# dmMaze/comic-text-detector

Hardware: AMD Instinct MI355X
Metric: pages/sec at 1024x1024 bs=32 (end-to-end detector, device-resident pages) (higher is better)
Workload: dtype f16

## Files before the change

comic-text-detector_amd/csrc/kernels.h:

```cpp
#pragma once
#include <vector>

#include "ctd_common.h"

void launch_conv_direct(const ConvArgs& a, bool f16, hipStream_t st);
void launch_convt_direct(const ConvArgs& a, bool f16, hipStream_t st);
void launch_input_nchw(const float* in, void* dst, int pitch, int B, int H, int W, bool f16, hipStream_t st);
void launch_input_u8(const uint8_t* in, void* dst, int pitch, int B, int H, int W, bool f16, hipStream_t st);
void launch_maxpool(const void* src, int pitchS, void* dst, int pitchD, int C, int B, int H, int W, int k,
                    bool f16, hipStream_t st);
bool sppf_pool3_supported(int pitch, int slot, int C, int H, int W, int k, const void* cat, int esize = 2);
void launch_sppf_pool3(void* cat, int pitch, int slot, int C, int B, int H, int W, int k, hipStream_t st, int esize = 2);
void launch_avgpool2(const void* src, int pitchS, void* dst, int pitchD, int C, int B, int Ho, int Wo,
                     bool f16, hipStream_t st);
void launch_detect_decode(const void* raw, int pitch, bool raw_f16, float* blks, int rows_total, int row_off,
                          int B, int ny, int nx, int na, int no, float stride, const float* anchors_px,
                          hipStream_t st);
void launch_export_plane(const void* src, int pitch, bool f16, float* out, int nplanes, int plane, uint8_t* u8,
                         int u8_mode, float thresh, int B, int H, int W, hipStream_t st);

void launch_db_step(const float* lines, float k, float* out, uint8_t* bitmap, float thresh, int B, int H, int W,
                    hipStream_t st);

extern int g_tail_max_blocks;
extern int g_igemm_force_bk;
int igemm_pick_bk(int c0, int c1, int K, int N, int log2_down);
void igemm_pack_weights(const float* logical, int nphase, int N, int K, int bn, int bk, bool tiled,
                        std::vector<half_t>& out);
bool igemm_supported(const ConvArgs& a);
int igemm_ntile(int N);
const char* launch_conv_igemm(const ConvArgs& a, bool dst_f32, hipStream_t st);

int f32_mfma_ntile(int N);
bool conv_f32_mfma_supported(const ConvArgs& a);
void launch_conv_f32_mfma(const ConvArgs& a, hipStream_t st);

bool conv_split_supported(const ConvArgs& a);
const char* launch_conv_split(const ConvArgs& a, hipStream_t st);
bool stem_split_supported(const ConvArgs& a);
void launch_stem_split(const ConvArgs& a, const void* input, int in_fmt, hipStream_t st);
extern int g_split_halo;
extern long long g_split_halo_min_patches;
bool conv_split_halo_supported(const ConvArgs& a);
void launch_conv_split_halo(const ConvArgs& a, hipStream_t st);
void split_pack_weights(const float* logical, int nphase, int N, int K, int npad, std::vector<half_t>& out,
                        std::vector<float>& oscale);

extern int g_conv_halo;
bool conv_halo_supported(const ConvArgs& a, bool dst_f32);
int conv_tuning_set(const char* key, long long value);
void launch_conv_halo(const ConvArgs& a, hipStream_t st);

extern long long g_halo3;
extern long long g_halo3_min_blocks;
bool conv_halo3_supported(const ConvArgs& a, bool dst_f32);
bool conv_halo3_post_supported(const ConvArgs& a);
bool conv_halo3_segp_supported(const ConvArgs& a);
void launch_conv_halo3(const ConvArgs& a, hipStream_t st);
int halo3_tuning_set(const char* key, long long value);

struct C3Args {
  SrcView s0, s1;
  int B, H, W;
  const half_t *w12, *wm1, *wm2, *wc3;
  const float *b12, *bm1, *bm2, *bc3;
  void* dst;
  int pitchD;
  int act;
  const void* zeros;
  int prio;
  half_t* dbg;
};
extern int g_fuse;
extern long long g_c3_min_patches;
bool c3_fused_supported(const C3Args& a);
void launch_c3_fused(const C3Args& a, hipStream_t st);

struct C3bArgs {
  SrcView y1;
  SrcView y2;
  int B, H, W;
  int ch;
  const half_t *wm1, *wm2, *wc3;
  const float *bm1, *bm2, *bc3;
  void* dst;
  int pitchD;
  int act;
  int add;
  int cv3;
  int tap_major;
  const void* zeros;
  int prio;
};
extern long long g_c3b_min_patches;
extern int g_c3b_max_ch;
extern int g_c3b_cfg64, g_c3b_cfg128;
bool c3b_supported(const C3bArgs& a);
const char* launch_c3b(const C3bArgs& a, hipStream_t st);

struct Stem2Args {
  const void* in; int in_fmt;
  int B, H, W;
  const half_t* wfrag; const float* bias0; int act0;
  const half_t* w1; const float* bias1; int act1;
  half_t* dst; int pitchD;
  int prio;
};
bool stem_conv2_supported(const Stem2Args& a);
void launch_stem_conv2(const Stem2Args& a, hipStream_t st);

void launch_stem(const void* in, int in_fmt, half_t* dst, int pitchD, int B, int H, int W, int N,
                 const half_t* wfrag, const float* bias, int act, hipStream_t st);
void stem_pack_weights(const float* W , std::vector<half_t>& out);
const char* launch_seg_final(const half_t* src, int pitch, int C, int B, int H, int W, const float* w, float bias,
                             float* mask, uint8_t* mask_u8, hipStream_t st);
void launch_seg_final_f32(const float* src, int pitch, int C, int B, int H, int W, const float* w, float* mask,
                          uint8_t* mask_u8, hipStream_t st);
void launch_seg_final_gather(const float* P, int B, int H, int W, float bias, float* mask, uint8_t* mask_u8, hipStream_t st);
extern int g_seg_final_mfma;
extern int g_db_up_mfma;
const char* launch_db_up(const void* src, bool f32in, int pitch, int q, int nbr, int B, int H, int W, const float* params,
                         float* lines, uint8_t* bitmap, float thresh, hipStream_t st);

size_t nms_workspace_bytes(int B, int rows);
void launch_nms(const float* blks, int B, int rows, int no, float conf, float iou, int max_det, int max_nms,
                float max_wh, float* dets, int* counts, void* ws, hipStream_t st);
size_t ccl_workspace_bytes(int B, int H, int W);
void launch_ccl(const uint8_t* img, int B, int H, int W, int thresh, int conn, int* labels, int* n_out,
                int* stats, int max_labels, void* ws, hipStream_t st, int invert = 0, int* first = nullptr, int bg_negative = 0);
void launch_ccl_dual(const uint8_t* img, int B, int H, int W, int thresh, int* labels, int* n_f, int* n_b, int* st_f,
                     int* st_b, int* first_f, int* first_b, int max_labels, void* ws, hipStream_t st);

void launch_resize_linear_u8(const uint8_t* src, int sH, int sW, int C, uint8_t* dst, int dH, int dW, int canvasH,
                             int canvasW, hipStream_t st);

void launch_region_warp(const ctd_region_job* jobs, int n, const int* tile_first, int n_tiles, uint8_t* out, hipStream_t st);
void launch_region_batches(const ctd_region_batch_job* jobs, int n, const int* tile_first, int n_tiles, const void* tables,
                           void* out, int dtype, int layout, int reverse, int pad, hipStream_t st);

void launch_mfma_probe(const half_t* a, const half_t* b, float* out, hipStream_t st);
```

comic-text-detector_amd/csrc/kernels_basic.hip:

```cpp
#include "kernels.h"

namespace {

template <typename T>
__device__ __forceinline__ const T* src_pixel(const SrcView& s, int b, int iy, int ix) {
  int sy = s.up ? (iy >> 1) : iy;
  int sx = s.up ? (ix >> 1) : ix;
  return (const T*)s.ptr + ((size_t)((size_t)b * s.H + sy) * s.W + sx) * s.pitch;
}

template <typename T, bool PRECISE>
__global__ __launch_bounds__(256) void conv_direct_kernel(ConvArgs a) {
  const long long total = (long long)a.M * a.N;
  const int Ct = a.s0.c + a.s1.c;
  const float* __restrict__ w = (const float*)a.w;
  for (long long idx = (long long)blockIdx.x * blockDim.x + threadIdx.x; idx < total;
       idx += (long long)gridDim.x * blockDim.x) {
    const int n = (int)(idx % a.N);
    const int m = (int)(idx / a.N);
    const int ox = m % a.Mw;
    const int oy = (m / a.Mw) % a.Mh;
    const int b = m / (a.Mw * a.Mh);
    float acc = 0.f;
    for (int ty = 0; ty < a.KH; ++ty) {
// ... 25 lines not shown
  const long long total = (long long)a.B * a.oH * a.oW * a.N;
  const int C = a.s0.c;
  const int k = a.KH, s = a.stride, p = a.dy0;
  const float* __restrict__ w = (const float*)a.w;
  for (long long idx = (long long)blockIdx.x * blockDim.x + threadIdx.x; idx < total;
       idx += (long long)gridDim.x * blockDim.x) {
    const int n = (int)(idx % a.N);
    const long long pix = idx / a.N;
    const int ox = (int)(pix % a.oW);
    const int oy = (int)((pix / a.oW) % a.oH);
    const int b = (int)(pix / ((long long)a.oW * a.oH));
    float acc = 0.f;
    for (int ky = 0; ky < k; ++ky) {
      const int ty = oy + p - ky;
      if (ty < 0 || (ty % s) != 0) continue;
      const int iy = ty / s;
      if (iy >= a.Hin) continue;
      for (int kx = 0; kx < k; ++kx) {
        const int tx = ox + p - kx;
        if (tx < 0 || (tx % s) != 0) continue;
        const int ix = tx / s;
        if (ix >= a.Win) continue;
        const T* p0 = src_pixel<T>(a.s0, b, iy, ix);
        const float* wp = w + (size_t)((ky * k + kx) * C) * a.N + n;
        for (int c = 0; c < C; ++c) acc = fmaf(to_f(p0[c]), wp[(size_t)c * a.N], acc);
      }
    }
    if (a.bias) acc += a.bias[n];
    acc = PRECISE ? ctd_act_precise(acc, a.act) : ctd_act(acc, a.act);
    ((T*)a.dst)[(size_t)pix * a.pitchD + n] = from_f<T>(acc);
  }
}

template <typename T>
__global__ void input_nchw_kernel(const float* __restrict__ in, T* __restrict__ dst, int pitch, int B, int H, int W) {
  const long long hw = (long long)H * W;
  const long long total = (long long)B * hw;
  for (long long i = (long long)blockIdx.x * blockDim.x + threadIdx.x; i < total;
       i += (long long)gridDim.x * blockDim.x) {
    const long long b = i / hw, p = i % hw;
    const float* src = in + b * 3 * hw + p;
    T* d = dst + i * pitch;
    d[0] = from_f<T>(src[0]);
    d[1] = from_f<T>(src[hw]);
    d[2] = from_f<T>(src[2 * hw]);
    for (int c = 3; c < pitch; ++c) d[c] = from_f<T>(0.f);
  }
}

template <typename T>
__global__ void input_u8_kernel(const uint8_t* __restrict__ in, T* __restrict__ dst, int pitch, long long total) {
  for (long long i = (long long)blockIdx.x * blockDim.x + threadIdx.x; i < total;
       i += (long long)gridDim.x * blockDim.x) {
    const uint8_t* s = in + i * 3;
    T* d = dst + i * pitch;
    d[0] = from_f<T>((float)s[0] / 255.0f);
    d[1] = from_f<T>((float)s[1] / 255.0f);
    d[2] = from_f<T>((float)s[2] / 255.0f);
    for (int c = 3; c < pitch; ++c) d[c] = from_f<T>(0.f);
  }
}

template <typename T>
__global__ void maxpool_kernel(const T* __restrict__ src, int pitchS, T* __restrict__ dst, int pitchD, int C,
                               int B, int H, int W, int k) {
  const long long total = (long long)B * H * W * C;
  const int r = k / 2;
  for (long long i = (long long)blockIdx.x * blockDim.x + threadIdx.x; i < total;
       i += (long long)gridDim.x * blockDim.x) {
    const int c = (int)(i % C);
    const long long pix = i / C;
    const int x = (int)(pix % W), y = (int)((pix / W) % H);
    const long long b = pix / ((long long)W * H);
    float m = -INFINITY;
    for (int dy = -r; dy <= r; ++dy) {
      const int yy = y + dy;
      if (yy < 0 || yy >= H) continue;
      for (int dx = -r; dx <= r; ++dx) {
        const int xx = x + dx;
        if (xx < 0 || xx >= W) continue;
        m = fmaxf(m, to_f(src[((b * H + yy) * W + xx) * pitchS + c]));
      }
    }
    dst[pix * pitchD + c] = from_f<T>(m);
  }
}

__global__ void maxpool_h8_kernel(const half_t* __restrict__ src, int pitchS, half_t* __restrict__ dst, int pitchD,
                                  int C8, int B, int H, int W, int k) {
  const long long total = (long long)B * H * W * C8;
  const int r = k / 2;
  for (long long i = (long long)blockIdx.x * blockDim.x + threadIdx.x; i < total;
       i += (long long)gridDim.x * blockDim.x) {
    const int c = (int)(i % C8) * 8;
    const long long pix = i / C8;
    const int x = (int)(pix % W), y = (int)((pix / W) % H);
    const long long b = pix / ((long long)W * H);
    half8_t m;
#pragma unroll
    for (int e = 0; e < 8; ++e) m[e] = (half_t)-65504.f;
    for (int dy = -r; dy <= r; ++dy) {
      const int yy = y + dy;
      if (yy < 0 || yy >= H) continue;
      for (int dx = -r; dx <= r; ++dx) {
        const int xx = x + dx;
        if (xx < 0 || xx >= W) continue;
        const half8_t v = *(const half8_t*)(src + ((b * H + yy) * W + xx) * pitchS + c);
#pragma unroll
        for (int e = 0; e < 8; ++e) m[e] = v[e] > m[e] ? v[e] : m[e];
      }
    }
    *(half8_t*)(dst + pix * pitchD + c) = m;
  }
}

constexpr int SPPF_LDS_BYTES = 65536;
template <typename T, typename V, int NV>
__global__ __launch_bounds__(256) void sppf_pool3_kernel(T* __restrict__ cat, int pitch, int slot, int CG, int H, int W, int r) {
  __shared__ __attribute__((aligned(16))) unsigned char sm_raw[SPPF_LDS_BYTES];
  V* A = (V*)sm_raw;
  V* Bf = A + H * W;
  const int HW = H * W;
  const int b = blockIdx.x / CG, cg = blockIdx.x - b * CG;
  T* base = cat + (size_t)b * HW * pitch + cg * NV;
  for (int p = threadIdx.x; p < HW; p += 256) A[p] = *(const V*)(base + (size_t)p * pitch);
  __syncthreads();
  auto vmax = [](V a, V b2) {
    V o;
#pragma unroll
    for (int e = 0; e < NV; ++e) o[e] = b2[e] > a[e] ? b2[e] : a[e];
    return o;
  };
  for (int lvl = 1; lvl <= 3; ++lvl) {
    for (int p = threadIdx.x; p < HW; p += 256) {
      const int y = p / W, x = p - y * W;
      V m = A[p];
      for (int dx = -r; dx <= r; ++dx)
        if (dx && (unsigned)(x + dx) < (unsigned)W) m = vmax(m, A[p + dx]);
      Bf[p] = m;
    }
    __syncthreads();
    for (int p = threadIdx.x; p < HW; p += 256) {
      const int y = p / W;
      V m = Bf[p];
      for (int dy = -r; dy <= r; ++dy)
        if (dy && (unsigned)(y + dy) < (unsigned)H) m = vmax(m, Bf[p + dy * W]);
      A[p] = m;
      *(V*)(base + (size_t)lvl * slot + (size_t)p * pitch) = m;
    }
    __syncthreads();
  }
}

template <typename T>
__global__ void avgpool2_kernel(const T* __restrict__ src, int pitchS, T* __restrict__ dst, int pitchD, int C,
                                int B, int Ho, int Wo) {
  const long long total = (long long)B * Ho * Wo * C;
  const int Wi = Wo * 2, Hi = Ho * 2;
  for (long long i = (long long)blockIdx.x * blockDim.x + threadIdx.x; i < total;
       i += (long long)gridDim.x * blockDim.x) {
    const int c = (int)(i % C);
    const long long pix = i / C;
    const int x = (int)(pix % Wo), y = (int)((pix / Wo) % Ho);
    const long long b = pix / ((long long)Wo * Ho);
    const T* p = src + ((b * Hi + 2 * y) * Wi + 2 * x) * pitchS + c;
    const float s = (to_f(p[0]) + to_f(p[pitchS])) + (to_f(p[(size_t)Wi * pitchS]) + to_f(p[(size_t)(Wi + 1) * pitchS]));
    dst[pix * pitchD + c] = from_f<T>(s * 0.25f);
  }
}

template <typename T>
__global__ void detect_decode_kernel(const T* __restrict__ raw, int pitch, float* __restrict__ blks, int rows_total,
                                     int row_off, int B, int ny, int nx, int na, int no, float stride,
                                     const float* __restrict__ anchors) {
  const long long total = (long long)B * na * ny * nx;
  for (long long i = (long long)blockIdx.x * blockDim.x + threadIdx.x; i < total;
       i += (long long)gridDim.x * blockDim.x) {
    const int x = (int)(i % nx), y = (int)((i / nx) % ny);
    const int an = (int)((i / ((long long)nx * ny)) % na);
    const long long b = i / ((long long)nx * ny * na);
    const T* p = raw + ((b * ny + y) * nx + x) * pitch + an * no;
    float* o = blks + (b * rows_total + row_off + ((long long)an * ny + y) * nx + x) * no;
    for (int j = 0; j < no; ++j) {
      const float s = 1.0f / (1.0f + expf(-to_f(p[j])));
      float v = s;
      if (j == 0) v = (s * 2.f - 0.5f + (float)x) * stride;
      else if (j == 1) v = (s * 2.f - 0.5f + (float)y) * stride;
      else if (j == 2) { const float t = s * 2.f; v = t * t * anchors[an * 2 + 0]; }
      else if (j == 3) { const float t = s * 2.f; v = t * t * anchors[an * 2 + 1]; }
      o[j] = v;
    }
  }
}

template <typename T>
__global__ void export_plane_kernel(const T* __restrict__ src, int pitch, float* __restrict__ out, int nplanes,
                                    int plane, uint8_t* __restrict__ u8, int u8_mode, float thresh, int B, int H,
                                    int W) {
  const long long hw = (long long)H * W;
  const long long total = (long long)B * hw;
  for (long long i = (long long)blockIdx.x * blockDim.x + threadIdx.x; i < total;
       i += (long long)gridDim.x * blockDim.x) {
    const long long b = i / hw, p = i % hw;
    const float v = to_f(src[i * pitch]);
    if (out) out[(b * nplanes + plane) * hw + p] = v;
    if (u8_mode == 1) u8[i] = (uint8_t)(v * 255.0f);
    else if (u8_mode == 2) u8[i] = v > thresh ? 1 : 0;
  }
}

inline int grid_for(long long total, int block = 256) {
  long long g = (total + block - 1) / block;
  if (g > 256LL * 32) g = 256LL * 32;
  if (g < 1) g = 1;
  return (int)g;
}

}

void launch_conv_direct(const ConvArgs& a, bool f16, hipStream_t st) {
  const int g = grid_for((long long)a.M * a.N);
  if (f16) hipLaunchKernelGGL((conv_direct_kernel<half_t, false>), dim3(g), dim3(256), 0, st, a);
  else hipLaunchKernelGGL((conv_direct_kernel<float, true>), dim3(g), dim3(256), 0, st, a);
}

void launch_convt_direct(const ConvArgs& a, bool f16, hipStream_t st) {
  const int g = grid_for((long long)a.B * a.oH * a.oW * a.N);
  if (f16) hipLaunchKernelGGL((convt_direct_kernel<half_t, false>), dim3(g), dim3(256), 0, st, a);
  else hipLaunchKernelGGL((convt_direct_kernel<float, true>), dim3(g), dim3(256), 0, st, a);
}

void launch_input_nchw(const float* in, void* dst, int pitch, int B, int H, int W, bool f16, hipStream_t st) {
  const int g = grid_for((long long)B * H * W);
  if (f16) hipLaunchKernelGGL((input_nchw_kernel<half_t>), dim3(g), dim3(256), 0, st, in, (half_t*)dst, pitch, B, H, W);
  else hipLaunchKernelGGL((input_nchw_kernel<float>), dim3(g), dim3(256), 0, st, in, (float*)dst, pitch, B, H, W);
}

void launch_input_u8(const uint8_t* in, void* dst, int pitch, int B, int H, int W, bool f16, hipStream_t st) {
  const long long t = (long long)B * H * W;
  const int g = grid_for(t);
  if (f16) hipLaunchKernelGGL((input_u8_kernel<half_t>), dim3(g), dim3(256), 0, st, in, (half_t*)dst, pitch, t);
  else hipLaunchKernelGGL((input_u8_kernel<float>), dim3(g), dim3(256), 0, st, in, (float*)dst, pitch, t);
}

void launch_maxpool(const void* src, int pitchS, void* dst, int pitchD, int C, int B, int H, int W, int k,
                    bool f16, hipStream_t st) {
  const int g = grid_for((long long)B * H * W * C);
  if (f16 && C % 8 == 0 && pitchS % 8 == 0 && pitchD % 8 == 0 && (((uintptr_t)src | (uintptr_t)dst) & 15) == 0)
    hipLaunchKernelGGL(maxpool_h8_kernel, dim3(grid_for((long long)B * H * W * (C / 8))), dim3(256), 0, st,
                       (const half_t*)src, pitchS, (half_t*)dst, pitchD, C / 8, B, H, W, k);
  else if (f16)
    hipLaunchKernelGGL((maxpool_kernel<half_t>), dim3(g), dim3(256), 0, st, (const half_t*)src, pitchS,
                       (half_t*)dst, pitchD, C, B, H, W, k);
  else
    hipLaunchKernelGGL((maxpool_kernel<float>), dim3(g), dim3(256), 0, st, (const float*)src, pitchS, (float*)dst,
                       pitchD, C, B, H, W, k);
}

bool sppf_pool3_supported(int pitch, int slot, int C, int H, int W, int k, const void* cat, int esize) {
  if (k != 5 && k != 3 && k != 7) return false;
  const int v = 16 / esize;
  if (C % v || pitch % v || slot % v || ((uintptr_t)cat & 15)) return false;
  return (long long)H * W * 2 * 8 <= SPPF_LDS_BYTES;
}
void launch_sppf_pool3(void* cat, int pitch, int slot, int C, int B, int H, int W, int k, hipStream_t st, int esize) {
  typedef float float2_t __attribute__((ext_vector_type(2)));
  const bool wide = (long long)H * W * 2 * 16 <= SPPF_LDS_BYTES;
  if (esize == 4) {
    if (wide)
      hipLaunchKernelGGL((sppf_pool3_kernel<float, float4_t, 4>), dim3(B * (C / 4)), dim3(256), 0, st, (float*)cat, pitch, slot, C / 4, H, W, k / 2);
    else
      hipLaunchKernelGGL((sppf_pool3_kernel<float, float2_t, 2>), dim3(B * (C / 2)), dim3(256), 0, st, (float*)cat, pitch, slot, C / 2, H, W, k / 2);
  } else if (wide) {
    hipLaunchKernelGGL((sppf_pool3_kernel<half_t, half8_t, 8>), dim3(B * (C / 8)), dim3(256), 0, st, (half_t*)cat, pitch, slot, C / 8, H, W, k / 2);
  } else {
    hipLaunchKernelGGL((sppf_pool3_kernel<half_t, half4_t, 4>), dim3(B * (C / 4)), dim3(256), 0, st, (half_t*)cat, pitch, slot, C / 4, H, W, k / 2);
  }
}

void launch_avgpool2(const void* src, int pitchS, void* dst, int pitchD, int C, int B, int Ho, int Wo, bool f16,
                     hipStream_t st) {
  const int g = grid_for((long long)B * Ho * Wo * C);
  if (f16)
    hipLaunchKernelGGL((avgpool2_kernel<half_t>), dim3(g), dim3(256), 0, st, (const half_t*)src, pitchS,
                       (half_t*)dst, pitchD, C, B, Ho, Wo);
  else
    hipLaunchKernelGGL((avgpool2_kernel<float>), dim3(g), dim3(256), 0, st, (const float*)src, pitchS, (float*)dst,
                       pitchD, C, B, Ho, Wo);
}

void launch_detect_decode(const void* raw, int pitch, bool raw_f16, float* blks, int rows_total, int row_off, int B,
                          int ny, int nx, int na, int no, float stride, const float* anchors_px, hipStream_t st) {
  const int g = grid_for((long long)B * na * ny * nx);
  if (raw_f16)
    hipLaunchKernelGGL((detect_decode_kernel<half_t>), dim3(g), dim3(256), 0, st, (const half_t*)raw, pitch, blks,
                       rows_total, row_off, B, ny, nx, na, no, stride, anchors_px);
  else
    hipLaunchKernelGGL((detect_decode_kernel<float>), dim3(g), dim3(256), 0, st, (const float*)raw, pitch, blks,
                       rows_total, row_off, B, ny, nx, na, no, stride, anchors_px);
}

__global__ void db_step_kernel(const float* __restrict__ lines, float k, float* __restrict__ out,
                               uint8_t* __restrict__ bitmap, float thresh, int B, int hw) {
  const long long total = (long long)B * hw;
  for (long long i = (long long)blockIdx.x * blockDim.x + threadIdx.x; i < total; i += (long long)gridDim.x * blockDim.x) {
    const long long b = i / hw, p = i % hw;
    const float x = lines[(b * 2) * hw + p], y = lines[(b * 2 + 1) * hw + p];
    const float v = 1.0f / (1.0f + expf(-k * (x - y)));
    out[i] = v;
    if (bitmap) bitmap[i] = v > thresh ? 1 : 0;
  }
}

void launch_db_step(const float* lines, float k, float* out, uint8_t* bitmap, float thresh, int B, int H, int W,
                    hipStream_t st) {
  hipLaunchKernelGGL(db_step_kernel, dim3(grid_for((long long)B * H * W)), dim3(256), 0, st, lines, k, out, bitmap, thresh,
                     B, H * W);
}

void launch_export_plane(const void* src, int pitch, bool f16, float* out, int nplanes, int plane, uint8_t* u8,
                         int u8_mode, float thresh, int B, int H, int W, hipStream_t st) {
  const int g = grid_for((long long)B * H * W);
  if (!u8) u8_mode = 0;
  if (f16)
    hipLaunchKernelGGL((export_plane_kernel<half_t>), dim3(g), dim3(256), 0, st, (const half_t*)src, pitch, out,
                       nplanes, plane, u8, u8_mode, thresh, B, H, W);
  else
    hipLaunchKernelGGL((export_plane_kernel<float>), dim3(g), dim3(256), 0, st, (const float*)src, pitch, out,
                       nplanes, plane, u8, u8_mode, thresh, B, H, W);
}
```

comic-text-detector_amd/csrc/selftest.hip:

```cpp
#include <cmath>
#include <cstdio>
#include <cstdlib>
#include <cstring>
#include <string>
#include <vector>

#include "kernels.h"

#define CK(x)                                                                              \
  do {                                                                                     \
    hipError_t e_ = (x);                                                                   \
    if (e_ != hipSuccess) {                                                                \
      std::printf("HIP error %s at %s:%d\n", hipGetErrorString(e_), __FILE__, __LINE__);   \
      std::exit(2);                                                                        \
    }                                                                                      \
  } while (0)

static unsigned g_seed = 12345;
static float frand() {
  static const bool zero = std::getenv("ST_ZERO") != nullptr;
  g_seed = g_seed * 1664525u + 1013904223u;
  return zero ? 0.f : ((g_seed >> 8) & 0xFFFF) / 65536.0f - 0.5f;
}

// ... 929 lines not shown
      CK(hipDeviceSynchronize());
      CK(hipMemcpy(o.data(), dOut, nout * 4, hipMemcpyDeviceToHost));
      for (size_t g = 0; g + 32 <= nout; g += 32) {
        half_t h[64];
        std::memcpy(h, &o[g], 128);
        for (int c = 0; c < 32; ++c) o[g + c] = (float)h[c] + (float)h[32 + c];
      }
      double maxd = 0;
      size_t bad = 0;
      for (size_t i = 0; i < nout; ++i) {
        const double e = std::fabs((double)o[i] - (double)r[i]);
        maxd = std::fmax(maxd, e / (1.0 + std::fabs((double)r[i])));
        if (!(e <= 2e-5 * (1.0 + std::fabs((double)r[i])))) ++bad;
      }
      double rms_s, mx_s;
      err64(o, rms_s, mx_s);
      const bool fail = bad || !(rms_s <= 3.0 * rms_f + 2e-7);
      if (fail) ++g_fail;
      const double ms_s = timing ? time_it([&]() { launch_conv_split(ap, 0); }) : 0;
      std::printf(halo ? " split(planes,halo):" : " split(planes):");
      std::printf(" %s err vs f64 rms %.2e max %.2e, max|d| vs f32-MFMA %.2e (%zu > 2e-5), %.3f ms %.0f TF %.0f GB/s |",
                  fail ? "FAIL" : "ok", rms_s, mx_s, maxd, bad, ms_s, flops / (ms_s * 1e-3) / 1e12, bytes / (ms_s * 1e-3) / 1e9);
      ConvArgs am = as;
      am.d_sp = 1;
      CK(hipMemset(dOut, 0xff, nout * 4));
      launch_conv_split(am, 0);
      CK(hipDeviceSynchronize());
      std::vector<float> o2(nout);
      CK(hipMemcpy(o2.data(), dOut, nout * 4, hipMemcpyDeviceToHost));
      size_t bad2 = 0;
      for (size_t g = 0; g + 32 <= nout; g += 32) {
        half_t h[64];
        std::memcpy(h, &o2[g], 128);
        for (int c = 0; c < 32; ++c) {
          const float v = (float)h[c] + (float)h[32 + c];
          if (!(std::fabs((double)v - (double)r[g + c]) <= 2e-5 * (1.0 + std::fabs((double)r[g + c])))) ++bad2;
        }
      }
      ConvArgs an = ap;
      an.d_sp = 0;
      CK(hipMemset(dOut, 0xff, nout * 4));
      launch_conv_split(an, 0);
      CK(hipDeviceSynchronize());
      CK(hipMemcpy(o2.data(), dOut, nout * 4, hipMemcpyDeviceToHost));
      size_t bad3 = 0;
      for (size_t i = 0; i < nout; ++i)
        if (!(std::fabs((double)o2[i] - (double)r[i]) <= 2e-5 * (1.0 + std::fabs((double)r[i])))) ++bad3;
      if (bad2 || bad3) ++g_fail;
      std::printf(" f32->planes %s, planes->f32 %s |", bad2 ? "FAIL" : "ok", bad3 ? "FAIL" : "ok");
     }
     g_split_halo = 1;
     g_split_halo_min_patches = minp;
    }
    (void)hipFree(d0s); (void)hipFree(d1s); if (dRs) (void)hipFree(dRs);
  }
  std::printf("\n");
  (void)hipFree(d0); (void)hipFree(d1); (void)hipFree(dOut); (void)hipFree(dRef); if (dRes) (void)hipFree(dRes);
  (void)hipFree(dWf); (void)hipFree(dWs); (void)hipFree(dBias); (void)hipFree(dOsc);
}

static void run_stem_split_case(int B, int H, bool timing) {
  const int W = H, Ho = H / 2, Wo = W / 2, N = 32, K = 144, Ks = 160;
  const size_t npx = (size_t)B * H * W;
  std::vector<uint8_t> img(npx * 3);
  for (auto& v : img) { g_seed = g_seed * 1664525u + 1013904223u; v = (uint8_t)(g_seed >> 24); }
  std::vector<float> planes(npx * 3);
  for (int b = 0; b < B; ++b)
    for (size_t p = 0; p < (size_t)H * W; ++p)
      for (int c = 0; c < 3; ++c) planes[((size_t)b * 3 + c) * H * W + p] = (float)img[((size_t)b * H * W + p) * 3 + c] / 255.0f;
  uint8_t* dImg = dev_alloc<uint8_t>(img.size());
  float *dPl = dev_alloc<float>(planes.size()), *dIn4 = dev_alloc<float>(npx * 4);
  CK(hipMemcpy(dImg, img.data(), img.size(), hipMemcpyHostToDevice));
  CK(hipMemcpy(dPl, planes.data(), planes.size() * 4, hipMemcpyHostToDevice));
  std::vector<float> lg((size_t)N * Ks, 0.f), bias(N);
  for (int n = 0; n < N; ++n) {
    const float ch = std::ldexp(1.f, (int)(frand() * 8.f) - 2);
    for (int tap = 0; tap < 36; ++tap)
      for (int c = 0; c < 3; ++c) lg[(size_t)n * Ks + tap * 4 + c] = frand() * 0.2f * ch;
    bias[n] = frand();
  }
  (void)K;
  std::vector<half_t> ws;
  std::vector<float> osc;
  split_pack_weights(lg.data(), 1, N, Ks, 32, ws, osc);
  half_t* dWs = dev_alloc<half_t>(ws.size());
  float *dBias = dev_alloc<float>(32), *dOsc = dev_alloc<float>(32);
  CK(hipMemcpy(dWs, ws.data(), ws.size() * 2, hipMemcpyHostToDevice));
  CK(hipMemcpy(dBias, bias.data(), 32 * 4, hipMemcpyHostToDevice));
  CK(hipMemcpy(dOsc, osc.data(), 32 * 4, hipMemcpyHostToDevice));
  const size_t nout = (size_t)B * Ho * Wo * N;
  float *dRef = dev_alloc<float>(nout), *dOut = dev_alloc<float>(nout);
  ConvArgs a{};
  a.s0 = SrcView{dIn4, 4, 4, 0, H, W};
  a.B = B; a.Hin = H; a.Win = W; a.Mh = Ho; a.Mw = Wo; a.KH = a.KW = 6; a.stride = 2; a.dy0 = a.dx0 = -2;
  a.bias = dBias; a.pitchD = N; a.oH = Ho; a.oW = Wo; a.act = CTD_ACT_SILU; a.N = N; a.Npad = 32; a.K = Ks; a.M = B * Ho * Wo;
  a.nphase = 1; a.osy = a.osx = 1;
  a.w = dWs; a.w2 = dWs + (size_t)32 * Ks; a.oscale = dOsc; a.dst = dRef;
  std::printf("[stem-split] %dx%dx%d -> %dx%dx32 |", B, H, W, Ho, Wo);
  if (!conv_split_supported(a) || !stem_split_supported(a)) { std::printf(" unsupported FAIL\n"); ++g_fail; return; }
  launch_input_u8(dImg, dIn4, 4, B, H, W, false, 0);
  launch_conv_split(a, 0);
  CK(hipDeviceSynchronize());
  std::vector<float> r(nout), o(nout);
  CK(hipMemcpy(r.data(), dRef, nout * 4, hipMemcpyDeviceToHost));
  ConvArgs an = a;
  an.dst = dOut;
  for (int var = 0; var < 3; ++var) {
    an.d_sp = var == 1;
    CK(hipMemset(dOut, 0xff, nout * 4));
    if (var == 2) launch_stem_split(an, dPl, CTD_IN_NCHW_F32, 0);
    else launch_stem_split(an, dImg, CTD_IN_NHWC_U8, 0);
    CK(hipDeviceSynchronize());
    CK(hipMemcpy(o.data(), dOut, nout * 4, hipMemcpyDeviceToHost));
    if (var == 1)
      for (size_t g = 0; g + 32 <= nout; g += 32) {
        half_t h[64];
        std::memcpy(h, &o[g], 128);
        for (int c = 0; c < 32; ++c) o[g + c] = (float)h[c] + (float)h[32 + c];
      }
    double maxd = 0;
    size_t bad = 0;
    for (size_t i = 0; i < nout; ++i) {
      const double e = std::fabs((double)o[i] - (double)r[i]);
      maxd = std::fmax(maxd, e / (1.0 + std::fabs((double)r[i])));
      if (!(e <= 2e-5 * (1.0 + std::fabs((double)r[i])))) ++bad;
    }
    if (bad) ++g_fail;
    std::printf(" %s: %s max|d| %.2e (%zu > 2e-5)", var == 0 ? "u8->f32" : var == 1 ? "u8->planes" : "nchw->f32", bad ? "FAIL" : "ok", maxd, bad);
  }
  if (timing) {
    hipEvent_t e0, e1;
    CK(hipEventCreate(&e0)); CK(hipEventCreate(&e1));
    auto tm = [&](auto&& fn) {
      for (int i = 0; i < 3; ++i) fn();
      CK(hipEventRecord(e0, 0));
      for (int i = 0; i < 20; ++i) fn();
      CK(hipEventRecord(e1, 0));
      CK(hipEventSynchronize(e1));
      float ms;
      CK(hipEventElapsedTime(&ms, e0, e1));
      return ms / 20;
    };
    an.d_sp = 1;
    const float t_new = tm([&]() { launch_stem_split(an, dImg, CTD_IN_NHWC_U8, 0); });
    const float t_old = tm([&]() { launch_input_u8(dImg, dIn4, 4, B, H, W, false, 0); launch_conv_split(a, 0); });
    std::printf(" | INPUT + generic %.3f ms, from the page %.3f ms (%.0f GB/s of its bytes)", t_old, t_new,
                ((double)npx * 3 + (double)nout * 4) / (t_new * 1e-3) / 1e9);
  }
  std::printf("\n");
  (void)hipFree(dImg); (void)hipFree(dPl); (void)hipFree(dIn4); (void)hipFree(dWs); (void)hipFree(dBias); (void)hipFree(dOsc);
  (void)hipFree(dRef); (void)hipFree(dOut);
}

int main(int argc, char** argv) {
  const int B = argc > 1 ? std::atoi(argv[1]) : 4;
  const bool quick = argc > 2;
  char name[256];
  int cus = 0;
  int64_t hbm = 0;
  const int arch = ctd_device_info(0, name, &cus, &hbm);
  std::printf("device: %s gfx%d CUs=%d HBM=%.1f GB\n", name, arch, cus, hbm / 1e9);
  if (const char* tu = std::getenv("CTD_TUNING")) {
    std::string s(tu);
    for (size_t p = 0; p < s.size();) {
      const size_t e = s.find(',', p), q = s.find('=', p);
      const size_t end = e == std::string::npos ? s.size() : e;
      if (q != std::string::npos && q < end) {
        const std::string k = s.substr(p, q - p);
        const long long v = std::atoll(s.substr(q + 1, end - q - 1).c_str());
        std::printf("tuning %s = %lld: %s\n", k.c_str(), v, ctd_tuning_set(k.c_str(), v) == CTD_OK ? "ok" : "UNKNOWN KEY");
      }
      p = end + 1;
    }
  }
  probe();
  const Case cases[] = {
      {"1x1 64->64 @256 (N64)", 0, 64, 0, 0, 64, 1, 1, 256, 0},
      {"1x1 32->32 @256 (N32)", 0, 32, 0, 0, 32, 1, 1, 256, 0},
      {"1x1 128->21 @128 detect (N21)", 0, 128, 0, 0, 21, 1, 1, 128, 0},
      {"1x1 256->256 @128", 0, 256, 0, 0, 256, 1, 1, 128, 0},
      {"1x1 512->512 @64", 0, 512, 0, 0, 512, 1, 1, 64, 0},
      {"1x1 cat(256up,256)->256 @64", 0, 256, 256, 1, 256, 1, 1, 64, 0},
      {"1x1 cat(512,256)->512 @32", 0, 512, 256, 0, 512, 1, 1, 32, 0},
      {"1x1 cat(128,256)->256 @128", 0, 128, 256, 0, 256, 1, 1, 128, 0},
      {"3x3 32->32 @256 +res", 0, 32, 0, 0, 32, 3, 1, 256, 1},
      {"3x3 64->64 @128 +res", 0, 64, 0, 0, 64, 3, 1, 128, 1},
      {"3x3 128->128 @128 +res", 0, 128, 0, 0, 128, 3, 1, 128, 1},
      {"3x3 256->256 @64 +res", 0, 256, 0, 0, 256, 3, 1, 64, 1},
      {"3x3 64->32 @256 (db tail)", 0, 64, 0, 0, 32, 3, 1, 256, 0},
      {"3x3s2 32->64 @512", 0, 32, 0, 0, 64, 3, 2, 512, 0},
      {"3x3s2 64->128 @256", 0, 64, 0, 0, 128, 3, 2, 256, 0},
      {"3x3s2 256->512 @64", 0, 256, 0, 0, 512, 3, 2, 64, 0},
      {"convT4 512->256 @64", 1, 512, 0, 0, 256, 4, 2, 64, 0},
      {"convT4 256->128 @128", 1, 256, 0, 0, 128, 4, 2, 128, 0},
      {"convT4 128->64 @256", 1, 128, 0, 0, 64, 4, 2, 256, 0},
      {"convT4 512->256 @16", 1, 512, 0, 0, 256, 4, 2, 16, 0},
  };
  const int ncase = sizeof(cases) / sizeof(cases[0]);
  if (std::getenv("ST_CORUN")) {
    run_stem2_case("1024x1024 pages", B, 1024, 1024, CTD_IN_NHWC_U8, CTD_ACT_SILU);
    std::printf("selftest: %s (%d failures)\n", g_fail ? "FAILED" : "PASSED", g_fail);
    return g_fail ? 1 : 0;
  }
  if (std::getenv("ST_SPLIT")) {
    probe_denorm();
    const Case ragged[] = {{"3x3 32->64 @20 ragged (s2)", 0, 32, 0, 0, 64, 3, 2, 20, 0},
                           {"1x1 cat(32up,64)->21 @12", 0, 32, 64, 1, 21, 1, 1, 12, 0},
                           {"convT4 64->32 @9", 1, 64, 0, 0, 32, 4, 2, 9, 0},
                           {"3x3 64->16 @24 (db branch)", 0, 64, 0, 0, 16, 3, 1, 24, 0},
                           {"stem 6x6s2 4->32 @44 ragged", 0, 4, 0, 0, 32, 6, 2, 44, 0},
                           {"3x3 64->64 @21 +res", 0, 64, 0, 0, 64, 3, 1, 21, 1},
                           {"3x3 cat(32,32)->128 @18 (halo)", 0, 32, 32, 0, 128, 3, 1, 18, 0},
                           {"convT4 64->64 @19 (halo)", 1, 64, 0, 0, 64, 4, 2, 19, 0},
                           {"convT4 96->128 @33 (halo)", 1, 96, 0, 0, 128, 4, 2, 33, 0}};
    for (const Case& c : ragged) run_split_case(c, 3, false);
    run_stem_split_case(3, 88, false);
    run_stem_split_case(B, 1024, true);
    run_split_case(Case{"stem 6x6s2 4->32 @1024", 0, 4, 0, 0, 32, 6, 2, 1024, 0}, B, true);
    const char* sel = std::getenv("ST_CASES");
    for (int i = 0; i < ncase; ++i) {
      if (sel) {
        bool on = false;
        for (const char* p = sel; *p;) {
          if (std::atoi(p) == i) on = true;
          while (*p && *p != ',') ++p;
          if (*p == ',') ++p;
        }
        if (!on) continue;
      }
      run_split_case(cases[i], B, true);
    }
    std::printf("selftest: %s (%d failures)\n", g_fail ? "FAILED" : "PASSED", g_fail);
    return g_fail ? 1 : 0;
  }
  if (!std::getenv("ST_NO_C3")) {
    const C3Case c3s[] = {{"model.2 (64 -> 64 @256)", 64, 0, 256, CTD_ACT_SILU},
                          {"upconv5.conv.0 (64+32 -> 64 @512)", 64, 32, 512, CTD_ACT_LEAKY},
                          {"two sources 32+32, relu @128", 32, 32, 128, CTD_ACT_RELU}};
    for (const C3Case& c : c3s) run_c3_case(c, B, c.H, c.H);
    run_c3_case(C3Case{"ragged 40x52 map (partial patches)", 64, 0, 0, CTD_ACT_SILU}, 3, 40, 52);
    run_c3_case(C3Case{"ragged 9x17 map, one source 96", 96, 0, 0, CTD_ACT_LEAKY}, 2, 9, 17);
    if (std::getenv("ST_C3_DBG")) {
      run_c3_case(C3Case{"64 leaky @128", 64, 0, 128, CTD_ACT_LEAKY}, B, 128, 128);
      run_c3_case(C3Case{"64 relu @128", 64, 0, 128, CTD_ACT_RELU}, B, 128, 128);
      run_c3_case(C3Case{"64 silu @128", 64, 0, 128, CTD_ACT_SILU}, B, 128, 128);
      run_c3_case(C3Case{"64+32 silu @128", 64, 32, 128, CTD_ACT_SILU}, B, 128, 128);
      run_c3_case(C3Case{"32 silu @128", 32, 0, 128, CTD_ACT_SILU}, B, 128, 128);
    }
    run_stem2_case("1024x1024 pages", B, 1024, 1024, CTD_IN_NHWC_U8, CTD_ACT_SILU);
    run_stem2_case("1024x1024 pages (float in)", B > 2 ? 2 : B, 1024, 1024, CTD_IN_NCHW_F32, CTD_ACT_SILU);
    run_stem2_case("192x320 (mostly border)", 3, 192, 320, CTD_IN_NHWC_U8, CTD_ACT_LEAKY);
    run_stem2_case("64x64 (all border)", 2, 64, 64, CTD_IN_NCHW_F32, CTD_ACT_RELU);
    run_sppf_case(B, 32, 32, 256);
    run_sppf_case(3, 48, 48, 256);
    run_sppf_case(2, 20, 36, 64);
    run_sppf_case(1, 72, 72, 256);
    run_dbup_case(B, 256, 256, 2);
    run_dbup_case(3, 40, 52, 1);
    run_dbup_case(1, 7, 9, 2);
    run_segfinal_case(B, 512, 512);
    run_segfinal_case(3, 40, 52);
    run_segfinal_case(2, 9, 17);
  }
  if (std::getenv("ST_ONLY_C3")) {
    std::printf("selftest: %s (%d failures)\n", g_fail ? "FAILED" : "PASSED", g_fail);
    return g_fail ? 1 : 0;
  }
  const char* sel = std::getenv("ST_CASES");
  for (int i = 0; i < ncase; ++i) {
    if (quick && i % 3) continue;
    if (sel) {
      bool on = false;
      for (const char* p = sel; *p;) {
        if (std::atoi(p) == i) on = true;
        while (*p && *p != ',') ++p;
        if (*p == ',') ++p;
      }
      if (!on) continue;
    }
    run_case(cases[i], B, true);
  }
  std::printf("selftest: %s (%d failures)\n", g_fail ? "FAILED" : "PASSED", g_fail);
  return g_fail ? 1 : 0;
}
```

Baseline: 3330.

## Add wide SPPF pool kernel, vectorized avgpool2, and LDS-staged detect decode

Adds a 1024-thread SPPF max-pool kernel that handles 32 channels per block with the whole small feature map held in LDS, reusing it across the three chained pools. Also adds a 16-byte vectorized f16 avgpool2 path and a detect-decode kernel that stages each 128-pixel chunk of raw outputs in LDS so global loads and stores are coalesced. These target small, latency-bound kernels in the neck and head. They add code paths gated on alignment and size, plus self-tests that check bit-identical output.

```diff
diff --git a/comic-text-detector_amd/csrc/kernels.h b/comic-text-detector_amd/csrc/kernels.h
--- a/comic-text-detector_amd/csrc/kernels.h
+++ b/comic-text-detector_amd/csrc/kernels.h
@@ -11,6 +11,8 @@
                     bool f16, hipStream_t st);
 bool sppf_pool3_supported(int pitch, int slot, int C, int H, int W, int k, const void* cat, int esize = 2);
 void launch_sppf_pool3(void* cat, int pitch, int slot, int C, int B, int H, int W, int k, hipStream_t st, int esize = 2);
+bool sppf_pool3_wide(int pitch, int slot, int C, int H, int W, int k, const void* cat, int esize = 2);
+extern int g_sppf_force_narrow;
 void launch_avgpool2(const void* src, int pitchS, void* dst, int pitchD, int C, int B, int Ho, int Wo,
                      bool f16, hipStream_t st);
 void launch_detect_decode(const void* raw, int pitch, bool raw_f16, float* blks, int rows_total, int row_off,
diff --git a/comic-text-detector_amd/csrc/kernels_basic.hip b/comic-text-detector_amd/csrc/kernels_basic.hip
--- a/comic-text-detector_amd/csrc/kernels_basic.hip
+++ b/comic-text-detector_amd/csrc/kernels_basic.hip
@@ -201,6 +201,68 @@
   }
 }
 
+constexpr int SPPF_WIDE_PIX = SPPF_LDS_BYTES / 64, SPPF_WIDE_NT = 1024, SPPF_WIDE_EPT = SPPF_WIDE_PIX * 4 / SPPF_WIDE_NT;
+template <int CH, int NT>
+__global__ __launch_bounds__(NT) void sppf_pool3_kernel(half_t* __restrict__ cat, int pitch, int slot, int CG, int H, int W, int r) {
+  static_assert(CH == 32, "four 16-B chunks per pixel");
+  __shared__ __attribute__((aligned(16))) half8_t A[SPPF_LDS_BYTES / 16];
+  const int HW4 = H * W * 4;
+  const int b = blockIdx.x / CG, cg = blockIdx.x - b * CG;
+  half_t* base = cat + (size_t)b * H * W * pitch + cg * CH;
+  auto vmax = [](half8_t a, half8_t b2) {
+    half8_t o;
+#pragma unroll
+    for (int e = 0; e < 8; ++e) o[e] = b2[e] > a[e] ? b2[e] : a[e];
+    return o;
+  };
+  int px[SPPF_WIDE_EPT], py[SPPF_WIDE_EPT];
+  size_t goff[SPPF_WIDE_EPT];
+  half8_t m[SPPF_WIDE_EPT];
+#pragma unroll
+  for (int i = 0; i < SPPF_WIDE_EPT; ++i) {
+    const int e = threadIdx.x + i * NT;
+    const int p = e >> 2;
+    py[i] = p / W;
+    px[i] = p - py[i] * W;
+    goff[i] = (size_t)p * pitch + (e & 3) * 8;
+    if (e < HW4) A[e] = *(const half8_t*)(base + goff[i]);
+  }
+  __syncthreads();
+  for (int lvl = 1; lvl <= 3; ++lvl) {
+#pragma unroll
+    for (int i = 0; i < SPPF_WIDE_EPT; ++i) {
+      const int e = threadIdx.x + i * NT;
+      if (e >= HW4) continue;
+      m[i] = A[e];
+      for (int dx = -r; dx <= r; ++dx)
+        if (dx && (unsigned)(px[i] + dx) < (unsigned)W) m[i] = vmax(m[i], A[e + dx * 4]);
+    }
+    __syncthreads();
+#pragma unroll
+    for (int i = 0; i < SPPF_WIDE_EPT; ++i) {
+      const int e = threadIdx.x + i * NT;
+      if (e < HW4) A[e] = m[i];
+    }
+    __syncthreads();
+#pragma unroll
+    for (int i = 0; i < SPPF_WIDE_EPT; ++i) {
+      const int e = threadIdx.x + i * NT;
+      if (e >= HW4) continue;
+      m[i] = A[e];
+      for (int dy = -r; dy <= r; ++dy)
+        if (dy && (unsigned)(py[i] + dy) < (unsigned)H) m[i] = vmax(m[i], A[e + dy * W * 4]);
+      *(half8_t*)(base + (size_t)lvl * slot + goff[i]) = m[i];
+    }
+    __syncthreads();
+#pragma unroll
+    for (int i = 0; i < SPPF_WIDE_EPT; ++i) {
+      const int e = threadIdx.x + i * NT;
+      if (e < HW4) A[e] = m[i];
+    }
+    __syncthreads();
+  }
+}
+
 template <typename T>
 __global__ void avgpool2_kernel(const T* __restrict__ src, int pitchS, T* __restrict__ dst, int pitchD, int C,
                                 int B, int Ho, int Wo) {
@@ -218,6 +280,42 @@
   }
 }
 
+template <int V>
+__global__ void avgpool2_kernel(const half_t* __restrict__ src, int pitchS, half_t* __restrict__ dst, int pitchD, int CV,
+                                int B, int Ho, int Wo) {
+  static_assert(V == 8, "16-B entries");
+  const long long total = (long long)B * Ho * Wo * CV;
+  const int Wi = Wo * 2, Hi = Ho * 2;
+  for (long long i = (long long)blockIdx.x * blockDim.x + threadIdx.x; i < total;
+       i += (long long)gridDim.x * blockDim.x) {
+    const int c = (int)(i % CV) * V;
+    const long long pix = i / CV;
+    const int x = (int)(pix % Wo), y = (int)((pix / Wo) % Ho);
+    const long long b = pix / ((long long)Wo * Ho);
+    const half_t* p = src + ((b * Hi + 2 * y) * Wi + 2 * x) * pitchS + c;
+    const half8_t p00 = *(const half8_t*)p, p01 = *(const half8_t*)(p + pitchS);
+    const half8_t p10 = *(const half8_t*)(p + (size_t)Wi * pitchS), p11 = *(const half8_t*)(p + (size_t)(Wi + 1) * pitchS);
+    half8_t o;
+#pragma unroll
+    for (int e = 0; e < V; ++e) {
+      const float s = (to_f(p00[e]) + to_f(p01[e])) + (to_f(p10[e]) + to_f(p11[e]));
+      o[e] = from_f<half_t>(s * 0.25f);
+    }
+    *(half8_t*)(dst + pix * pitchD + c) = o;
+  }
+}
+
+__device__ __forceinline__ float detect_decode_elem(float raw, int j, int x, int y, int an, float stride,
+                                                    const float* __restrict__ anchors) {
+  const float s = 1.0f / (1.0f + expf(-raw));
+  float v = s;
+  if (j == 0) v = (s * 2.f - 0.5f + (float)x) * stride;
+  else if (j == 1) v = (s * 2.f - 0.5f + (float)y) * stride;
+  else if (j == 2) { const float t = s * 2.f; v = t * t * anchors[an * 2 + 0]; }
+  else if (j == 3) { const float t = s * 2.f; v = t * t * anchors[an * 2 + 1]; }
+  return v;
+}
+
 template <typename T>
 __global__ void detect_decode_kernel(const T* __restrict__ raw, int pitch, float* __restrict__ blks, int rows_total,
                                      int row_off, int B, int ny, int nx, int na, int no, float stride,
@@ -230,14 +328,43 @@
     const long long b = i / ((long long)nx * ny * na);
     const T* p = raw + ((b * ny + y) * nx + x) * pitch + an * no;
     float* o = blks + (b * rows_total + row_off + ((long long)an * ny + y) * nx + x) * no;
-    for (int j = 0; j < no; ++j) {
-      const float s = 1.0f / (1.0f + expf(-to_f(p[j])));
-      float v = s;
-      if (j == 0) v = (s * 2.f - 0.5f + (float)x) * stride;
-      else if (j == 1) v = (s * 2.f - 0.5f + (float)y) * stride;
-      else if (j == 2) { const float t = s * 2.f; v = t * t * anchors[an * 2 + 0]; }
-      else if (j == 3) { const float t = s * 2.f; v = t * t * anchors[an * 2 + 1]; }
-      o[j] = v;
+    for (int j = 0; j < no; ++j) o[j] = detect_decode_elem(to_f(p[j]), j, x, y, an, stride, anchors);
+  }
+}
+
+constexpr int DEC_PIX = 128, DEC_PITCH_MAX = 32;
+template <typename T, int NO>
+__global__ __launch_bounds__(256) void detect_decode_kernel(const T* __restrict__ raw, int pitch, float* __restrict__ blks,
+                                                            int rows_total, int row_off, int nchunk, int ny, int nx, int na,
+                                                            int no_rt, float stride, const float* __restrict__ anchors, int vec) {
+  typedef unsigned int u32x4_t __attribute__((ext_vector_type(4)));
+  __shared__ __attribute__((aligned(16))) T s_raw[DEC_PIX * DEC_PITCH_MAX];
+  __shared__ int s_x[DEC_PIX], s_y[DEC_PIX];
+  const int no = NO ? NO : no_rt;
+  const int t = threadIdx.x;
+  const int b = blockIdx.x / nchunk, p0 = (blockIdx.x - b * nchunk) * DEC_PIX;
+  const int HW = ny * nx;
+  const int np = HW - p0 < DEC_PIX ? HW - p0 : DEC_PIX;
+  const T* src = raw + ((size_t)b * HW + p0) * pitch;
+  const int nel = np * pitch;
+  if (vec) {
+    constexpr int VE = 16 / (int)sizeof(T);
+    for (int i = t; i < nel / VE; i += 256) ((u32x4_t*)s_raw)[i] = ((const u32x4_t*)src)[i];
+  } else {
+    for (int i = t; i < nel; i += 256) s_raw[i] = src[i];
+  }
+  if (t < np) {
+    const int y = (p0 + t) / nx;
+    s_y[t] = y;
+    s_x[t] = p0 + t - y * nx;
+  }
+  __syncthreads();
+  const int nout = np * no;
+  for (int an = 0; an < na; ++an) {
+    float* o = blks + ((size_t)b * rows_total + row_off + (size_t)an * HW + p0) * no;
+    for (int i = t; i < nout; i += 256) {
+      const int px = i / no, j = i - px * no;
+      o[i] = detect_decode_elem(to_f(s_raw[px * pitch + an * no + j]), j, s_x[px], s_y[px], an, stride, anchors);
     }
   }
 }
@@ -312,8 +439,18 @@
   if (C % v || pitch % v || slot % v || ((uintptr_t)cat & 15)) return false;
   return (long long)H * W * 2 * 8 <= SPPF_LDS_BYTES;
 }
+int g_sppf_force_narrow = 0;
+bool sppf_pool3_wide(int pitch, int slot, int C, int H, int W, int k, const void* cat, int esize) {
+  if (g_sppf_force_narrow || esize != 2 || !sppf_pool3_supported(pitch, slot, C, H, W, k, cat, esize)) return false;
+  return C % 32 == 0 && (long long)H * W <= SPPF_WIDE_PIX;
+}
 void launch_sppf_pool3(void* cat, int pitch, int slot, int C, int B, int H, int W, int k, hipStream_t st, int esize) {
   typedef float float2_t __attribute__((ext_vector_type(2)));
+  if (sppf_pool3_wide(pitch, slot, C, H, W, k, cat, esize)) {
+    hipLaunchKernelGGL((sppf_pool3_kernel<32, SPPF_WIDE_NT>), dim3(B * (C / 32)), dim3(SPPF_WIDE_NT), 0, st, (half_t*)cat, pitch, slot,
+                       C / 32, H, W, k / 2);
+    return;
+  }
   const bool wide = (long long)H * W * 2 * 16 <= SPPF_LDS_BYTES;
   if (esize == 4) {
     if (wide)
@@ -330,7 +467,10 @@
 void launch_avgpool2(const void* src, int pitchS, void* dst, int pitchD, int C, int B, int Ho, int Wo, bool f16,
                      hipStream_t st) {
   const int g = grid_for((long long)B * Ho * Wo * C);
-  if (f16)
+  if (f16 && C % 8 == 0 && pitchS % 8 == 0 && pitchD % 8 == 0 && (((uintptr_t)src | (uintptr_t)dst) & 15) == 0)
+    hipLaunchKernelGGL((avgpool2_kernel<8>), dim3(grid_for((long long)B * Ho * Wo * (C / 8))), dim3(256), 0, st,
+                       (const half_t*)src, pitchS, (half_t*)dst, pitchD, C / 8, B, Ho, Wo);
+  else if (f16)
     hipLaunchKernelGGL((avgpool2_kernel<half_t>), dim3(g), dim3(256), 0, st, (const half_t*)src, pitchS,
                        (half_t*)dst, pitchD, C, B, Ho, Wo);
   else
@@ -340,6 +480,19 @@
 
 void launch_detect_decode(const void* raw, int pitch, bool raw_f16, float* blks, int rows_total, int row_off, int B,
                           int ny, int nx, int na, int no, float stride, const float* anchors_px, hipStream_t st) {
+  const int esize = raw_f16 ? 2 : 4;
+  const long long nchunk = ((long long)ny * nx + DEC_PIX - 1) / DEC_PIX;
+  if (pitch <= DEC_PITCH_MAX && na * no <= pitch && B * nchunk < (1LL << 31)) {
+    const int vec = (pitch * esize) % 16 == 0 && ((uintptr_t)raw & 15) == 0;
+    const dim3 grid((unsigned)(B * nchunk));
+#define CTD_DECODE(T, NO)                                                                                          \
+  hipLaunchKernelGGL((detect_decode_kernel<T, NO>), grid, dim3(256), 0, st, (const T*)raw, pitch, blks, rows_total, \
+                     row_off, (int)nchunk, ny, nx, na, no, stride, anchors_px, vec)
+    if (raw_f16) { if (no == 7) CTD_DECODE(half_t, 7); else CTD_DECODE(half_t, 0); }
+    else { if (no == 7) CTD_DECODE(float, 7); else CTD_DECODE(float, 0); }
+#undef CTD_DECODE
+    return;
+  }
   const int g = grid_for((long long)B * na * ny * nx);
   if (raw_f16)
     hipLaunchKernelGGL((detect_decode_kernel<half_t>), dim3(g), dim3(256), 0, st, (const half_t*)raw, pitch, blks,
diff --git a/comic-text-detector_amd/csrc/selftest.hip b/comic-text-detector_amd/csrc/selftest.hip
--- a/comic-text-detector_amd/csrc/selftest.hip
+++ b/comic-text-detector_amd/csrc/selftest.hip
@@ -1105,6 +1105,144 @@
   (void)hipFree(dRef); (void)hipFree(dOut);
 }
 
+static void run_sm_sppf_case(int B, int H, int W, int C, int k) {
+  const size_t n = (size_t)B * H * W * 4 * C;
+  std::vector<half_t> h(n);
+  for (auto& v : h) v = (half_t)frand();
+  half_t* d[3];
+  for (auto& p : d) { p = dev_alloc<half_t>(n); CK(hipMemcpy(p, h.data(), n * 2, hipMemcpyHostToDevice)); }
+  for (int j = 0; j < 3; ++j) launch_maxpool(d[0] + j * C, 4 * C, d[0] + (j + 1) * C, 4 * C, C, B, H, W, k, true, 0);
+  const bool sup = sppf_pool3_supported(4 * C, C, C, H, W, k, d[2]);
+  const bool wide = sppf_pool3_wide(4 * C, C, C, H, W, k, d[2]);
+  if (sup) {
+    g_sppf_force_narrow = 1;
+    launch_sppf_pool3(d[1], 4 * C, C, C, B, H, W, k, 0);
+    g_sppf_force_narrow = 0;
+    launch_sppf_pool3(d[2], 4 * C, C, C, B, H, W, k, 0);
+  }
+  CK(hipDeviceSynchronize());
+  std::vector<half_t> o[3];
+  for (int i = 0; i < 3; ++i) { o[i].resize(n); CK(hipMemcpy(o[i].data(), d[i], n * 2, hipMemcpyDeviceToHost)); }
+  const bool eq_kept = sup && std::memcmp(o[2].data(), o[1].data(), n * 2) == 0;
+  const bool eq_chain = sup && std::memcmp(o[2].data(), o[0].data(), n * 2) == 0;
+  if (!sup || !eq_kept || !eq_chain) ++g_fail;
+  std::printf("[sm-sppf] B=%d %dx%d C=%d k=%d | layout %s | vs kept kernel: %s | vs chained pools: %s\n", B, H, W, C, k,
+              !sup ? "unsupported" : wide ? "wide" : "kept", eq_kept ? "bit-identical" : "DIFFERENT", eq_chain ? "bit-identical" : "DIFFERENT");
+  for (auto& p : d) (void)hipFree(p);
+}
+
+template <typename T> __device__ __forceinline__ float st_to_f(T v) { return (float)v; }
+template <typename T>
+__global__ void ref_avgpool2_kernel(const T* __restrict__ src, int pitchS, T* __restrict__ dst, int pitchD, int C,
+                                    int B, int Ho, int Wo) {
+  const long long total = (long long)B * Ho * Wo * C;
+  const int Wi = Wo * 2, Hi = Ho * 2;
+  for (long long i = (long long)blockIdx.x * blockDim.x + threadIdx.x; i < total;
+       i += (long long)gridDim.x * blockDim.x) {
+    const int c = (int)(i % C);
+    const long long pix = i / C;
+    const int x = (int)(pix % Wo), y = (int)((pix / Wo) % Ho);
+    const long long b = pix / ((long long)Wo * Ho);
+    const T* p = src + ((b * Hi + 2 * y) * Wi + 2 * x) * pitchS + c;
+    const float s = (st_to_f(p[0]) + st_to_f(p[pitchS])) + (st_to_f(p[(size_t)Wi * pitchS]) + st_to_f(p[(size_t)(Wi + 1) * pitchS]));
+    dst[pix * pitchD + c] = (T)(s * 0.25f);
+  }
+}
+template <typename T>
+__global__ void ref_detect_decode_kernel(const T* __restrict__ raw, int pitch, float* __restrict__ blks, int rows_total,
+                                         int row_off, int B, int ny, int nx, int na, int no, float stride,
+                                         const float* __restrict__ anchors) {
+  const long long total = (long long)B * na * ny * nx;
+  for (long long i = (long long)blockIdx.x * blockDim.x + threadIdx.x; i < total;
+       i += (long long)gridDim.x * blockDim.x) {
+    const int x = (int)(i % nx), y = (int)((i / nx) % ny);
+    const int an = (int)((i / ((long long)nx * ny)) % na);
+    const long long b = i / ((long long)nx * ny * na);
+    const T* p = raw + ((b * ny + y) * nx + x) * pitch + an * no;
+    float* o = blks + (b * rows_total + row_off + ((long long)an * ny + y) * nx + x) * no;
+    for (int j = 0; j < no; ++j) {
+      const float s = 1.0f / (1.0f + expf(-st_to_f(p[j])));
+      float v = s;
+      if (j == 0) v = (s * 2.f - 0.5f + (float)x) * stride;
+      else if (j == 1) v = (s * 2.f - 0.5f + (float)y) * stride;
+      else if (j == 2) { const float t = s * 2.f; v = t * t * anchors[an * 2 + 0]; }
+      else if (j == 3) { const float t = s * 2.f; v = t * t * anchors[an * 2 + 1]; }
+      o[j] = v;
+    }
+  }
+}
+static int st_grid(long long total) { return (int)std::min<long long>(std::max<long long>((total + 255) / 256, 1), 256LL * 32); }
+
+static void run_sm_avgpool_case(int B, int Ho, int Wo, int C, int pitchS, int pitchD) {
+  const size_t ns = (size_t)B * 4 * Ho * Wo * pitchS, nd = (size_t)B * Ho * Wo * pitchD;
+  std::vector<half_t> h(ns);
+  for (auto& v : h) v = (half_t)(frand() * 8.f);
+  half_t *dS = dev_alloc<half_t>(ns), *dR = dev_alloc<half_t>(nd), *dO = dev_alloc<half_t>(nd);
+  CK(hipMemcpy(dS, h.data(), ns * 2, hipMemcpyHostToDevice));
+  CK(hipMemset(dR, 0xee, nd * 2));
+  CK(hipMemset(dO, 0xee, nd * 2));
+  hipLaunchKernelGGL((ref_avgpool2_kernel<half_t>), dim3(st_grid((long long)B * Ho * Wo * C)), dim3(256), 0, 0, dS, pitchS, dR, pitchD, C, B, Ho, Wo);
+  launch_avgpool2(dS, pitchS, dO, pitchD, C, B, Ho, Wo, true, 0);
+  CK(hipDeviceSynchronize());
+  std::vector<half_t> r(nd), o(nd);
+  CK(hipMemcpy(r.data(), dR, nd * 2, hipMemcpyDeviceToHost));
+  CK(hipMemcpy(o.data(), dO, nd * 2, hipMemcpyDeviceToHost));
+  const bool eq = std::memcmp(r.data(), o.data(), nd * 2) == 0;
+  if (!eq) ++g_fail;
+  std::printf("[sm-avgpool] B=%d out %dx%d C=%d pitch %d -> %d | %s | vs reference copy: %s\n", B, Ho, Wo, C, pitchS, pitchD,
+              C % 8 == 0 && pitchS % 8 == 0 && pitchD % 8 == 0 ? "16-B lanes" : "scalar", eq ? "bit-identical" : "DIFFERENT");
+  (void)hipFree(dS); (void)hipFree(dR); (void)hipFree(dO);
+}
+
+template <typename T>
+static void run_sm_decode_case(int B, int ny, int nx, int row_off, int extra_rows) {
+  const int na = 3, no = 7, pitch = 24;
+  const int rows_total = row_off + na * ny * nx + extra_rows;
+  const size_t nr = (size_t)B * ny * nx * pitch, nb = (size_t)B * rows_total * no;
+  std::vector<T> h(nr);
+  for (auto& v : h) v = (T)(frand() * 16.f);
+  const float anchors[6] = {10.f, 13.f, 16.f, 30.f, 33.f, 23.f};
+  T* dRaw = dev_alloc<T>(nr);
+  float *dA = dev_alloc<float>(6), *dR = dev_alloc<float>(nb), *dO = dev_alloc<float>(nb);
+  CK(hipMemcpy(dRaw, h.data(), nr * sizeof(T), hipMemcpyHostToDevice));
+  CK(hipMemcpy(dA, anchors, sizeof(anchors), hipMemcpyHostToDevice));
+  CK(hipMemset(dR, 0xee, nb * 4));
+  CK(hipMemset(dO, 0xee, nb * 4));
+  hipLaunchKernelGGL((ref_detect_decode_kernel<T>), dim3(st_grid((long long)B * na * ny * nx)), dim3(256), 0, 0, dRaw, pitch, dR, rows_total,
+                     row_off, B, ny, nx, na, no, 8.f, dA);
+  launch_detect_decode(dRaw, pitch, sizeof(T) == 2, dO, rows_total, row_off, B, ny, nx, na, no, 8.f, dA, 0);
+  CK(hipDeviceSynchronize());
+  std::vector<float> r(nb), o(nb);
+  CK(hipMemcpy(r.data(), dR, nb * 4, hipMemcpyDeviceToHost));
+  CK(hipMemcpy(o.data(), dO, nb * 4, hipMemcpyDeviceToHost));
+  const bool eq = std::memcmp(r.data(), o.data(), nb * 4) == 0;
+  if (!eq) ++g_fail;
+  std::printf("[sm-decode] %s B=%d grid %dx%d rows %d..%d of %d | vs reference copy: %s\n", sizeof(T) == 2 ? "f16" : "f32", B, ny, nx,
+              row_off, row_off + na * ny * nx, rows_total, eq ? "bit-identical" : "DIFFERENT");
+  (void)hipFree(dRaw); (void)hipFree(dA); (void)hipFree(dR); (void)hipFree(dO);
+}
+
+static void run_small_maps() {
+  const int maps[4][2] = {{2, 2}, {4, 10}, {32, 32}, {48, 48}};
+  for (const auto& m : maps)
+    for (int C : {256, 32}) run_sm_sppf_case(2, m[0], m[1], C, 5);
+  run_sm_sppf_case(2, 4, 10, 40, 5);
+  run_sm_sppf_case(2, 32, 32, 32, 3);
+  run_sm_sppf_case(2, 4, 10, 256, 7);
+  const int omaps[3][2] = {{1, 1}, {3, 5}, {16, 16}};
+  for (const auto& m : omaps) {
+    run_sm_avgpool_case(2, m[0], m[1], 512, 528, 520);
+    run_sm_avgpool_case(2, m[0], m[1], 8, 8, 8);
+    run_sm_avgpool_case(2, m[0], m[1], 12, 12, 12);
+  }
+  const int grids[5][2] = {{1, 1}, {2, 2}, {5, 3}, {32, 32}, {13, 11}};
+  for (const auto& g : grids)
+    for (int B : {1, 3}) {
+      run_sm_decode_case<float>(B, g[0], g[1], B == 1 ? 0 : 11, B == 1 ? 0 : 5);
+      run_sm_decode_case<half_t>(B, g[0], g[1], B == 1 ? 7 : 0, 3);
+    }
+}
+
 int main(int argc, char** argv) {
   const int B = argc > 1 ? std::atoi(argv[1]) : 4;
   const bool quick = argc > 2;
@@ -1125,6 +1263,11 @@
       }
       p = end + 1;
     }
+  }
+  if (std::getenv("ST_SMALL_MAPS")) {
+    run_small_maps();
+    std::printf("selftest: %s (%d failures)\n", g_fail ? "FAILED" : "PASSED", g_fail);
+    return g_fail ? 1 : 0;
   }
   probe();
   const Case cases[] = {
```

Measured after the change: 3299. About the same (-0.9%).
